# ArbiterMob/FluidSimulationCuda

Measured on AMD Instinct MI355X. Metric: Mcells/s per Jacobi iter, higher is better.
Workload: dtype f32

## Files before the change

### fluidsimulationcuda_amd/capi.py

```python
import ctypes as C
import os

import numpy as np

from ._build import LIB

OK, E_INVALID, E_NOMEM, E_HIP, E_COMM = 0, 1, 2, 3, 4
U, V, DENS, U_PREV, V_PREV, DENS_PREV, TMP0, TMP1, TMP2, TMP3, TMP4, TMP5 = range(12)
NFIELDS = 12
JACOBI_STREAM, JACOBI_LDS, JACOBI_NAIVE, JACOBI_TB = 0, 1, 2, 3
STORAGE_F32, STORAGE_F16 = 0, 1
PARAM_TB_MAX_SWEEPS, PARAM_TB_ROWS, PARAM_HALO, PARAM_TB_FAST_DIVISION, PARAM_TB_MIN_CELLS, PARAM_TB_EDGE_ROWS_PCT = 0, 1, 2, 3, 4, 5
PARAM_TB_LANE_COLUMNS = 6
PARAM_TB_T16_MIN_CELLS = 7
PARAM_TB_AUTOTUNE = 8
PARAM_FUSE_DIVERGENCE = 9
PARAM_SLAB_OVERLAP = 10
PARAM_EARLY_ADVECT = 11
PARAM_FUSE_ADD_SOURCE = 12
PARAM_XCHG_OVERLAP = 13
PARAM_F16_PRESSURE_SCALE = 14
XCHG_HALO, XCHG_GATHER, XCHG_MAX, XCHG_MAX_BEGIN, XCHG_MAX_END = 0, 1, 2, 3, 4
RCCL_ID_BYTES = 128
FIELD_NAMES = ("u", "v", "dens", "u_prev", "v_prev", "dens_prev", "tmp0", "tmp1", "tmp2", "tmp3", "tmp4", "tmp5")


class FluidError(RuntimeError):
    def __init__(self, code, msg):
        super().__init__("libfluid_amd error %d: %s" % (code, msg))
        self.code = code


class Config(C.Structure):
    _fields_ = [("n", C.c_int), ("rank", C.c_int), ("nranks", C.c_int), ("halo", C.c_int),
                ("jacobi_variant", C.c_int), ("stream", C.c_void_p), ("arena", C.c_void_p),
                ("arena_bytes", C.c_size_t), ("storage", C.c_int)]


TIME_SOURCE, TIME_DIFFUSION, TIME_DIVERGENCE, TIME_PROJECTION, TIME_ADVECTION = range(5)
TIMING_CATEGORIES = ("source", "diffusion", "divergence", "projection", "advection")


class Timing(C.Structure):
    _fields_ = [("jacobi_ms", C.c_double), ("sweeps", C.c_longlong), ("solves", C.c_longlong),
                ("category_ms", C.c_double * 5), ("category_calls", C.c_longlong * 5),
                ("jacobi_launches", C.c_longlong), ("jacobi_field_launches", C.c_longlong),
                ("pressure_ms", C.c_double), ("pressure_sweeps", C.c_longlong)]


EXCHANGE_FN = C.CFUNCTYPE(C.c_int, C.c_void_p, C.c_int, C.POINTER(C.c_int), C.c_int, C.c_int,
                          C.POINTER(C.c_float))

_HOSTF = np.ctypeslib.ndpointer(dtype=np.float32, flags="C_CONTIGUOUS")
_ctx = C.c_void_p
# ... 82 lines not shown
```

### fluidsimulationcuda_amd/csrc/fluid_ctx.h

```cpp
#pragma once
#include <hip/hip_runtime.h>

#include <string>
#include <vector>

#include "../../include/fluid_amd.h"
#include "fluid_kernels.h"

namespace fluid_detail {
int fail(int code, const char* fmt, ...);
int materialize_zero(fluid_ctx* c, int f);
struct RcclExchange;
void rccl_release(RcclExchange* x);
}

#define HIP_TRY(expr)                                                                                      \
    do {                                                                                                   \
        hipError_t e_ = (expr);                                                                            \
        if (e_ != hipSuccess)                                                                              \
            return fluid_detail::fail(e_ == hipErrorOutOfMemory ? FLUID_E_NOMEM : FLUID_E_HIP, "%s: %s",   \
                                      #expr, hipGetErrorString(e_));                                       \
    } while (0)

#define TRY(expr)                        \
// ... 14 lines not shown
};

struct fluid_ctx {
    int n = 0, w = 0, pitch = 0;
    size_t field_floats = 0;
    char* arena = nullptr;
    bool own_arena = false;
    int st = fluid::STORAGE_F32;
    size_t esz = 4;
    hipStream_t stream = nullptr;
    bool own_stream = false;
    hipStream_t stream2 = nullptr;
    hipEvent_t ev_fork = nullptr, ev_join = nullptr;
    bool slab_overlap = true;
    hipStream_t xstream = nullptr;
    hipEvent_t ev_xbegin = nullptr, ev_xdone = nullptr;
    bool xchg_overlap = true;
    unsigned xowed = 0;
    long long split_launches = 0;
    bool early_advect = true;
    float vmax_prev[2] = {-1.0f, -1.0f};
    FieldState field[FLUID_NFIELDS];
    size_t field_bytes = 0;
    unsigned int* d_scalar = nullptr;
    float* d_partials = nullptr;
    unsigned int* tiles = nullptr;
    unsigned int* h_scalar = nullptr;
    hipEvent_t scalar_ready = nullptr;
    int variant = fluid::JACOBI_TB;
    int tb_max_t = 16, tb_rows = 0, num_cu = 256;
    long long tb_min_cells = 0;
    long long tb_t16_min_cells = -1;
    bool fuse_divergence = true;
    bool autotune = true;
    struct Trial { unsigned long long key; int cand; hipEvent_t a, b; };
    std::vector<Trial> trials;
    std::vector<hipEvent_t> free_events;
    bool defer_zero_source = true;
    bool in_halo_exchange = false;
    int tb_nv = 2;
    int tb_edge_pct = 40;
    int fast_div = 2;
    int rank = 0, nranks = 1, own0 = 1, own1 = 1, min_slab = 0, halo = 1;
    bool fuse_add_source = true;
    float pscale = 1.0f;
    fluid_exchange_fn xchg = nullptr;
    void* xchg_user = nullptr;
    fluid_detail::RcclExchange* rccl = nullptr;
    bool timing = false;
    struct Ev { hipEvent_t a, b; int cat; bool pressure; };
    std::vector<Ev> ev_pool;
    size_t ev_used = 0;
    double cat_ms[FLUID_TIMING_CATEGORIES] = {};
    long long cat_calls[FLUID_TIMING_CATEGORIES] = {};
    long long sweeps = 0, pending_sweeps = 0, launches = 0, field_launches = 0;
    double pressure_ms = 0.0;
    long long pressure_sweeps = 0, pending_pressure_sweeps = 0;
    bool in_pressure_solve = false;

    bool valid_field(int id) const { return id >= 0 && id < FLUID_NFIELDS; }
    void* ptr(int id) const { return field[id].ptr; }
    void* row(int id, int r) const { return static_cast<char*>(ptr(id)) + (size_t)r * pitch * esz; }
    int lo_all() const { return own0 - (rank == 0 ? 1 : 0); }
    int hi_all() const { return own1 + (rank == nranks - 1 ? 1 : 0); }
};

// ... 1 lines not shown
```

### fluidsimulationcuda_amd/csrc/fluid_kernels.h

```cpp
#pragma once
#include <hip/hip_runtime.h>

namespace fluid {

constexpr int XOFF = 63;

enum JacobiVariant { JACOBI_STREAM = 0, JACOBI_LDS = 1, JACOBI_NAIVE = 2, JACOBI_TB = 3, JACOBI_VARIANTS = 4 };

enum Storage { STORAGE_F32 = 0, STORAGE_F16 = 1 };
typedef _Float16 half_t;
inline size_t storage_bytes(int st) { return st == STORAGE_F16 ? 2 : 4; }

inline int pitch_for(int n) { return ((XOFF + 1 + 4 * ((n + 3) / 4) + 1) + 63) / 64 * 64; }

struct TbBatch {
    const void* x[3];
    const void* x0[3];
    void* out[3];
    float alpha[3], beta[3];
    double yd[3];
    float hi[3], lo[3];
    const unsigned* tiles[3];
    unsigned tile_thr[3];
    int tile_pitch;
    void* div[3];
    float div_scale;
    int b[3];
    int x_zero[3];
    float x0_inc[3];
    int count;
};

void launch_set_bnd(hipStream_t s, int st, void* f, int pitch, int n, int b);
void launch_add_source(hipStream_t s, int st, void* x, const void* src, int pitch, int row_lo, int row_hi, float dt);
void launch_jacobi(hipStream_t s, int st, int variant, const void* x, const void* x0, void* out, int pitch, int n,
                   int row_lo, int row_hi, float alpha, float beta, int b);
void launch_jacobi_tb(hipStream_t s, int st, int T, int divmode, int nv, const TbBatch& batch, int pitch, int n, int row_lo,
                      int row_hi, int rb, int rb_edge, bool divsrc = false, bool addsrc = false, int hole_lo = 0, int hole_hi = 0);
inline bool jacobi_tb_addsrc_exists(int T, int divmode, int nv) { return nv == 2 && (T == 8 || T == 12 || T == 16) && (divmode == 0 || divmode == 2 || divmode == 5); }
constexpr int kTileRows = 32, kTileCols = 64;
inline int tile_rows(int n) { return (n + kTileRows - 1) / kTileRows; }
inline int tile_pitch(int n) { return (n + kTileCols - 1) / kTileCols; }
struct TileBatch {
    const void* field[3];
    unsigned* tiles[3];
};
void launch_tile_min_abs(hipStream_t s, int st, const TileBatch& tb, int count, int pitch, int n, int row_lo, int row_hi, int tile_pitch);
void launch_validate_div(hipStream_t s, int divmode, float beta, float kbeta, double yd, float hi, float lo, unsigned long long* bad);
void launch_advect(hipStream_t s, int st, void* d, const void* d0, const void* u, const void* v, int pitch, int n,
                   int row_lo, int row_hi, float dt0, int b);
void launch_advect2(hipStream_t s, int st, void* da, const void* d0a, int ba, void* db, const void* d0b, int bb, const void* u,
                    const void* v, int pitch, int n, int row_lo, int row_hi, float dt0);
void launch_divergence(hipStream_t s, int st, const void* u, const void* v, void* p, void* div, int pitch, int n,
                       int row_lo, int row_hi, float h, int write_p, float pscale = 1.0f);
void launch_scale(hipStream_t s, int st, void* x, int pitch, int row_lo, int row_hi, float factor);
constexpr int kMaxPartials = 8192;
void launch_subtract_gradient(hipStream_t s, int st, void* u, void* v, const void* p, int pitch, int n, int row_lo,
                              int row_hi, float h, float* partials = nullptr, unsigned int* max_out = nullptr, float pinv = 1.0f);
void launch_gradient_advect(hipStream_t s, int st, void* u, void* v, const void* p, void* d, const void* d0, int pitch, int n,
                            int row_lo, int row_hi, float h, float dt0, int b, float pinv = 1.0f);
void launch_absmax2(hipStream_t s, int st, const void* u, const void* v, int pitch, int n, int row_lo, int row_hi,
                    unsigned int* result);
void launch_residual(hipStream_t s, int st, const void* x, const void* x0, int pitch, int n, int row_lo, int row_hi,
                     float alpha, float beta, unsigned int* result);

}
```

### fluidsimulationcuda_amd/csrc/fluid_kernels.hip

```cpp
#include <hip/hip_runtime.h>
#include <stdint.h>

#include <algorithm>
#include <cstdlib>

#include "fluid_kernels.h"

namespace fluid {

__device__ __forceinline__ float flip_if(bool c, float v) { return c ? -v : v; }

__device__ __forceinline__ float keep_f32(float v) { asm("" : "+v"(v)); return v; }
__device__ __forceinline__ float ld1(const float* p) { return *p; }
__device__ __forceinline__ float ld1(const half_t* p) { return keep_f32((float)*p); }
__device__ __forceinline__ void st1(float* p, float v) { *p = v; }
__device__ __forceinline__ void st1(half_t* p, float v) { *p = (half_t)keep_f32(v); }
template <typename S>
__device__ __forceinline__ float as_stored(float v)
{
    if constexpr (sizeof(S) == 2) return keep_f32((float)(S)keep_f32(v));
    else return v;
}
typedef half_t half4_t __attribute__((ext_vector_type(4)));
__device__ __forceinline__ float4 ld4(const float* p) { return *reinterpret_cast<const float4*>(p); }
// ... 342 lines not shown
        __builtin_memcpy(&u, &h, 4);
        __builtin_amdgcn_raw_buffer_store_b32(u, r, off, 0, 0);
    }
}

struct DivK {
    float beta;
    double yd;
    float hi, lo;
};
constexpr float kDiv5NegScale = -0x1p24f;

template <typename S, int NV>
struct TbArgs {
    const S* xc;
    const S* rc;
    S* oc;
    __amdgpu_buffer_rsrc_t bx, br, bo;
    unsigned ld_off;
    unsigned st_off;
    unsigned row_bytes;
    unsigned m_lg;
    unsigned m_r[NV];
    int n, q_lo, q_hi, cg;
    float alpha;
    DivK k;
    S* dc;
    __amdgpu_buffer_rsrc_t bd;
    float div_scale;
    int s_lo, s_hi;
    unsigned sx, sy;
    float x0_inc;
    bool st_rg_lane, is_lg;
};

__device__ __forceinline__ float fxor(float v, unsigned m) { return __uint_as_float(__float_as_uint(v) ^ m); }
template <int NV>
__device__ __forceinline__ Vec<NV> fxorv(const Vec<NV>& v, unsigned m)
{
    Vec<NV> o;
#pragma unroll
    for (int c = 0; c < NV; ++c) o.c[c] = fxor(v.c[c], m);
    return o;
}

template <int DIVMODE>
__device__ __forceinline__ float tb_div(float num, const DivK& k)
{
    if (DIVMODE == 0) return num / k.beta;
    if (DIVMODE == 4) return num * k.beta;
    if (DIVMODE == 3) return __builtin_fmaf(num, k.hi, num * k.lo);
    if (DIVMODE == 5) {
        const float q0 = num * k.beta;
        const float e = __builtin_fmaf(q0, k.hi, num * kDiv5NegScale);
        return __builtin_fmaf(e, k.lo, q0);
    }
    return (float)((double)num * k.yd);
}
template <int DIVMODE>
__device__ __forceinline__ v2f tb_div2(v2f num, const DivK& k)
{
    if constexpr (DIVMODE == 4) return num * k.beta;
    else if constexpr (DIVMODE == 3) {
        const v2f p = num * k.lo;
        return __builtin_elementwise_fma(num, (v2f){k.hi, k.hi}, p);
    } else if constexpr (DIVMODE == 5) {
// ... 130 lines not shown

template <int NV>
__device__ __forceinline__ Vec<NV> take(const Vec<NV>& v)
{
    Vec<NV> o;
#pragma unroll
    for (int p = 0; p < NV; p += 2) {
        v2f in = {v.c[p], v.c[p + 1]}, out;
        asm("v_mov_b64 %0, %1" : "=v"(out) : "v"(in));
        o.c[p] = out.x;
        o.c[p + 1] = out.y;
    }
    return o;
}

template <int K, int N, int NV>
__device__ __forceinline__ void tb_qshift(Vec<NV> (&Q)[N])
{
    if constexpr (K >= 1) {
        Q[K] = Q[K - 1];
        tb_qshift<K - 1, N, NV>(Q);
    }
}

template <int DIVMODE, int NV>
__device__ __forceinline__ void tb_sticky(const Vec<NV>& G, v2f& nf)
{
    if constexpr (DIVMODE == 5) {
#pragma unroll
        for (int p = 0; p < NV; p += 2) nf = __builtin_elementwise_fma((v2f){G.c[p], G.c[p + 1]}, (v2f){0.f, 0.f}, nf);
    }
}

template <int T, int DIVMODE, bool EDGE, bool WALL, bool GEN, int PH, typename S, int NV, bool DIVSRC = false, bool ADDSRC = false>
__device__ __forceinline__ void tb_step(int t, Vec<NV> (&W)[T][3], Vec<NV> (&Q)[T + 1], Vec<NV> (&PX)[3], Vec<NV> (&PQ)[3],
                                        const TbArgs<S, NV>& a, Vec<NV> (&UR)[3], Vec<NV> (&VR)[3], v2f& nf)
{
    constexpr int UP = PH % 3, ME = (PH + 1) % 3, FR = (PH + 2) % 3;
    __builtin_amdgcn_sched_barrier(0);
    if constexpr (DIVSRC) {
        UR[FR] = take<NV>(PX[PH]);
        VR[FR] = take<NV>(PQ[PH]);
    } else {
        W[0][FR] = take<NV>(PX[PH]);
        Q[0] = take<NV>(PQ[PH]);
        if constexpr (ADDSRC) {
#pragma unroll
            for (int p = 0; p < NV; p += 2) {
                const v2f ds = (v2f){W[0][FR].c[p], W[0][FR].c[p + 1]} * a.div_scale;
                const v2f q = (v2f){Q[0].c[p], Q[0].c[p + 1]} + ds;
                Q[0].c[p] = as_stored<S>(q.x);
                Q[0].c[p + 1] = as_stored<S>(q.y);
            }
            buf_stv<NV>(a.dc, a.bd, (((t >= a.s_lo) & (t < a.s_hi)) ? a.st_off : kBufOff) + (unsigned)t * a.row_bytes, Q[0]);
        } else {
#pragma unroll
            for (int p = 0; p < NV; p += 2) {
                const v2f q = (v2f){Q[0].c[p], Q[0].c[p + 1]} + a.x0_inc;
                Q[0].c[p] = q.x;
                Q[0].c[p + 1] = q.y;
            }
        }
    }
    {
        const unsigned off = a.ld_off + (unsigned)(t + 3) * a.row_bytes;
        PX[PH] = buf_ldv<NV>(a.xc, a.bx, off);
        PQ[PH] = buf_ldv<NV>(a.rc, a.br, off);
    }
    __builtin_amdgcn_sched_barrier(0);
    if constexpr (DIVSRC) {
        const int q = t - 1;
        Vec<NV> D = tb_divergence<NV>(UR[ME], VR[UP], VR[FR], a.div_scale);
#pragma unroll
        for (int c = 0; c < NV; ++c) D.c[c] = as_stored<S>(D.c[c]);
        Q[1] = D;
        float v1 = 0.f, vn = 0.f;
        if (EDGE) tb_fix_columns<S, NV>(D, a, v1, vn, WALL);
        tb_store_to<EDGE, (WALL || GEN), S, NV>(a.dc, a.bd, D, q, (q >= 1) & (q <= a.n) & (q >= a.q_lo) & (q < a.q_hi), a, v1, vn);
    }
    if constexpr (!GEN) {
#pragma unroll
        for (int s = 1; s <= T; ++s) {
            const int q = t - s;
            Vec<NV> G = tb_stencil<DIVMODE, NV>(W[s - 1][UP], W[s - 1][ME], W[s - 1][FR], Q[s], a.alpha, a.k);
            float v1 = 0.f, vn = 0.f;
            if (EDGE) tb_fix_columns<S, NV>(G, a, v1, vn, WALL && s == T);
            if (s < T) W[s][FR] = G;
            else {
                tb_sticky<DIVMODE, NV>(G, nf);
                tb_store<EDGE, WALL, S, NV>(G, q, (q >= a.q_lo) & (q < a.q_hi), a, v1, vn);
            }
        }
    } else {
#pragma unroll
        for (int s = 1; s <= T; ++s) {
            const int q = t - s;
            const bool interior = (q >= 1 && q <= a.n);
            Vec<NV> G = tb_stencil<DIVMODE, NV>(W[s - 1][UP], W[s - 1][ME], W[s - 1][FR], Q[s], a.alpha, a.k);
            float v1 = 0.f, vn = 0.f;
            if (EDGE) tb_fix_columns<S, NV>(G, a, v1, vn, s == T);
            if (s < T) {
                const Vec<NV> me = W[s][ME];
                const Vec<NV> flipped_me = fxorv<NV>(me, a.sy);
                const Vec<NV> flipped_g = fxorv<NV>(G, a.sy);
                const bool bot_ghost = (q == a.n + 1), top_ghost = (q == 1);
#pragma unroll
                for (int c = 0; c < NV; ++c) {
                    W[s][FR].c[c] = bot_ghost ? flipped_me.c[c] : G.c[c];
                    W[s][ME].c[c] = top_ghost ? flipped_g.c[c] : me.c[c];
                }
            } else {
                tb_sticky<DIVMODE, NV>(G, nf);
                tb_store<EDGE, true, S, NV>(G, q, interior & (q >= a.q_lo) & (q < a.q_hi), a, v1, vn);
            }
        }
    }
    tb_qshift<T, T + 1, NV>(Q);
}

template <int T, int DIVMODE, bool EDGE, bool WALL, typename S, int NV, bool DIVSRC = false, bool ADDSRC = false>
__device__ __forceinline__ bool tb_march(int t0, int t1, const TbArgs<S, NV>& a)
{
    Vec<NV> W[T][3], Q[T + 1], PX[3], PQ[3], UR[3], VR[3];
    v2f nf = {0.f, 0.f};
    Vec<NV> zero;
#pragma unroll
    for (int c = 0; c < NV; ++c) zero.c[c] = 0.f;
#pragma unroll
    for (int s = 0; s < T; ++s) { W[s][0] = zero; W[s][1] = zero; W[s][2] = zero; }
#pragma unroll
    for (int s = 0; s <= T; ++s) Q[s] = zero;
#pragma unroll
    for (int d = 0; d < 3; ++d) { UR[d] = zero; VR[d] = zero; }
#pragma unroll
    for (int d = 0; d < 3; ++d) {
        const unsigned off = a.ld_off + (unsigned)(t0 + d) * a.row_bytes;
        PX[d] = buf_ldv<NV>(a.xc, a.bx, off);
        PQ[d] = buf_ldv<NV>(a.rc, a.br, off);
        buf_stv<NV>(a.oc, a.bo, kBufOff, zero);
        if constexpr (DIVSRC || ADDSRC) buf_stv<NV>(a.dc, a.bd, kBufOff, zero);
        __builtin_amdgcn_sched_barrier(0);
    }
    int t = t0;
    if constexpr (WALL) {
        for (; t <= t1 && t < T + 1; t += 3) {
            tb_step<T, DIVMODE, EDGE, WALL, true, 0, S, NV, DIVSRC, ADDSRC>(t, W, Q, PX, PQ, a, UR, VR, nf);
            tb_step<T, DIVMODE, EDGE, WALL, true, 1, S, NV, DIVSRC, ADDSRC>(t + 1, W, Q, PX, PQ, a, UR, VR, nf);
            tb_step<T, DIVMODE, EDGE, WALL, true, 2, S, NV, DIVSRC, ADDSRC>(t + 2, W, Q, PX, PQ, a, UR, VR, nf);
        }
    }
    for (; t <= t1 && (!WALL || t + 1 <= a.n); t += 3) {
        tb_step<T, DIVMODE, EDGE, WALL, false, 0, S, NV, DIVSRC, ADDSRC>(t, W, Q, PX, PQ, a, UR, VR, nf);
        tb_step<T, DIVMODE, EDGE, WALL, false, 1, S, NV, DIVSRC, ADDSRC>(t + 1, W, Q, PX, PQ, a, UR, VR, nf);
        tb_step<T, DIVMODE, EDGE, WALL, false, 2, S, NV, DIVSRC, ADDSRC>(t + 2, W, Q, PX, PQ, a, UR, VR, nf);
    }
    if constexpr (WALL) {
        for (; t <= t1; t += 3) {
            tb_step<T, DIVMODE, EDGE, WALL, true, 0, S, NV, DIVSRC, ADDSRC>(t, W, Q, PX, PQ, a, UR, VR, nf);
            tb_step<T, DIVMODE, EDGE, WALL, true, 1, S, NV, DIVSRC, ADDSRC>(t + 1, W, Q, PX, PQ, a, UR, VR, nf);
            tb_step<T, DIVMODE, EDGE, WALL, true, 2, S, NV, DIVSRC, ADDSRC>(t + 2, W, Q, PX, PQ, a, UR, VR, nf);
        }
    }
    if constexpr (DIVMODE == 5) return __builtin_amdgcn_ballot_w64((nf.x != nf.x) | (nf.y != nf.y)) != 0ull;
    else return false;
}

template <int T, int DIVMODE, typename S, int NV, bool DIVSRC = false, bool ADDSRC = false>
__device__ __forceinline__ bool tb_march_any(bool edge, bool wall, int t0, int t1, const TbArgs<S, NV>& a)
{
    if (edge) {
        if (wall) return tb_march<T, DIVMODE, true, true, S, NV, DIVSRC, ADDSRC>(t0, t1, a);
        return tb_march<T, DIVMODE, true, false, S, NV, DIVSRC, ADDSRC>(t0, t1, a);
    }
    if (wall) return tb_march<T, DIVMODE, false, true, S, NV, DIVSRC, ADDSRC>(t0, t1, a);
    return tb_march<T, DIVMODE, false, false, S, NV, DIVSRC, ADDSRC>(t0, t1, a);
}

struct TbGrid {
    int inner_wins, inner_blocks, edge_wins, edge_blocks, first_right;
    int hole_lo, hole_hi;
};

constexpr int tb_waves_per_simd(int T, int NV) { return NV == 2 ? (T <= 8 ? 4 : T <= 12 ? 3 : 2) : (T <= 4 ? 3 : 2); }

template <int T, int DIVMODE, int NV, typename S, bool DIVSRC = false, bool ADDSRC = false>
__global__ __launch_bounds__(256, tb_waves_per_simd(T, NV)) void k_jacobi_tb(TbBatch batch, int pitch, int n, int row_lo,
                                                                             int row_hi, int rb, int rb_edge, TbGrid g)
{
    static_assert(!DIVSRC || DIVMODE == 4, "the divergence-sourced launch is the first launch of a pressure solve");
    static_assert(!(DIVSRC && ADDSRC) && (!ADDSRC || DIVMODE != 3), "one second store per launch; mode 3's tiles are taken from the summed field");
    const unsigned per_xcd = gridDim.x >> 3;
    unsigned vid = (blockIdx.x & 7u) * per_xcd + (blockIdx.x >> 3);
    if (vid >= (unsigned)(g.inner_blocks + g.edge_blocks)) return;
    int win, strip_group;
    if (vid < (unsigned)g.inner_blocks) {
        win = 1 + (int)(vid % (unsigned)g.inner_wins);
        strip_group = (int)(vid / (unsigned)g.inner_wins);
    } else {
        vid -= (unsigned)g.inner_blocks;
        const int e = (int)(vid % (unsigned)g.edge_wins);
        strip_group = (int)(vid / (unsigned)g.edge_wins);
        win = e == 0 ? 0 : g.first_right + e - 1;
    }
    const S* __restrict__ x = static_cast<const S*>(batch.x[blockIdx.z]);
    const S* __restrict__ x0 = static_cast<const S*>(batch.x0[blockIdx.z]);
    S* __restrict__ out = static_cast<S*>(batch.out[blockIdx.z]);
    const float alpha = batch.alpha[blockIdx.z], beta = batch.beta[blockIdx.z];
    const double yd = batch.yd[blockIdx.z];
    const int b = batch.b[blockIdx.z];
    constexpr int HL = (T + NV - 1) / NV;
    constexpr int VS = 64 - 2 * HL;
    constexpr int C0 = (XOFF + 1) / NV;
    static_assert((XOFF + 1) % NV == 0 && HL <= C0, "window overlap must fit the row's left pad");
    const int lane = threadIdx.x & 63;
    const int strip = strip_group * 4 + __builtin_amdgcn_readfirstlane(threadIdx.x >> 6);
    const int kg = n / NV;
    const bool left_edge = (win == 0);
    const bool right_edge = (kg >= win * VS - HL) && (kg < win * VS - HL + 64);
    const bool edge = left_edge || right_edge;
    const int rbw = edge ? rb_edge : rb;
// ... 18 lines not shown
    const bool ld_ok = k <= pitch / NV - C0 - 1;
    const ptrdiff_t cofs = (ptrdiff_t)(XOFF + 1) + NV * (ptrdiff_t)(ld_ok ? k : 0);
    a.xc = x + cofs;
    a.rc = x0 + cofs;
    a.oc = out + cofs;
    {
        const unsigned field_bytes = (unsigned)((size_t)(n + 2) * (size_t)pitch * sizeof(S));
        a.bx = __builtin_amdgcn_make_buffer_rsrc(const_cast<S*>(x), 0, (batch.x_zero[blockIdx.z] && !DIVSRC) ? 0u : field_bytes, 0x00020000);
        a.br = __builtin_amdgcn_make_buffer_rsrc(const_cast<S*>(x0), 0, field_bytes, 0x00020000);
        a.bo = __builtin_amdgcn_make_buffer_rsrc(out, 0, field_bytes, 0x00020000);
        S* dv = (DIVSRC || ADDSRC) ? static_cast<S*>(batch.div[blockIdx.z]) : out;
        a.dc = dv + cofs;
        a.bd = __builtin_amdgcn_make_buffer_rsrc(dv, 0, field_bytes, 0x00020000);
        a.div_scale = batch.div_scale;
        a.row_bytes = (unsigned)((size_t)pitch * sizeof(S));
        const unsigned col = (unsigned)((XOFF + 1 + NV * (ptrdiff_t)k) * (ptrdiff_t)sizeof(S));
        a.ld_off = ld_ok ? col : kBufOff;
    }
    a.n = n;
    a.cg = n % NV;
    a.is_lg = (k == -1);
    const bool is_rg = (k == kg);
    const bool own = (lane >= HL) && (lane < 64 - HL);
    const bool st_int = own && k >= 0 && k < nvec;
    a.st_rg_lane = is_rg && (own || k == nvec);
    a.m_lg = a.is_lg ? 0xFFFFFFFFu : 0u;
#pragma unroll
    for (int c = 0; c < NV; ++c) a.m_r[c] = (is_rg && a.cg == c) ? 0xFFFFFFFFu : 0u;
    a.st_off = (ld_ok && (st_int || a.is_lg || a.st_rg_lane)) ? a.ld_off : kBufOff;
    a.sx = (b == 1) ? 0x80000000u : 0u;
    a.sy = (b == 2) ? 0x80000000u : 0u;
    a.alpha = alpha;
    a.k.beta = beta;
    const int t0 = max(0, a.q_lo - T), t1 = a.q_hi - 1 + T;
    const bool wall = (a.q_lo < T) || (a.q_hi - 1 + T > n + 1);
    constexpr int DM = DIVMODE == 3 ? 2 : DIVMODE;
    bool two_term = false;
    if constexpr (DIVMODE == 3) {
        const unsigned* __restrict__ tiles = batch.tiles[blockIdx.z];
        const unsigned thr = batch.tile_thr[blockIdx.z];
        const int tr0 = (max(1, a.q_lo - T + 1) - 1) / kTileRows, tr1 = (min(n, a.q_hi + T - 2) - 1) / kTileRows;
        const int c0 = max(1, 1 + NV * (win * VS - HL)), c1 = min(n, NV * (win * VS - HL + 64));
        const int tc0 = (c0 - 1) / kTileCols, tc1 = (c1 - 1) / kTileCols, ntc = tc1 - tc0 + 1;
        const int count = (tr1 - tr0 + 1) * ntc;
        bool low = false;
        if (tiles != nullptr)
            for (int i = lane; i < count; i += 64)
                low |= tiles[(size_t)(tr0 + i / ntc) * batch.tile_pitch + (tc0 + i % ntc)] < thr;
        two_term = tiles != nullptr && __builtin_amdgcn_ballot_w64(low) == 0ull;
    }
    if (two_term) {
        tb_march_any<T, DIVMODE, S, NV>(edge, wall, t0, t1, a);
    } else {
        const bool again = tb_march_any<T, DM, S, NV, DIVSRC, ADDSRC>(edge, wall, t0, t1, a);
        if constexpr (DIVMODE == 5) {
            if (again) tb_march_any<T, 2, S, NV, false, ADDSRC>(edge, wall, t0, t1, a);
        }
    }
}

template <typename S>
__global__ __launch_bounds__(256) void k_tile_min_abs(TileBatch tb, int pitch, int n, int row_lo, int row_hi, int tile_row0, int tile_pitch)
{
    const S* __restrict__ f = static_cast<const S*>(tb.field[blockIdx.z]);
    unsigned* __restrict__ out = tb.tiles[blockIdx.z];
    const int lane = threadIdx.x & 63, wave = threadIdx.x >> 6;
// ... 392 lines not shown
{
    const size_t total = (size_t)(row_hi - row_lo) * (pitch >> 2);
    const unsigned blocks = (unsigned)((total + 255) / 256 < 8192 ? (total + 255) / 256 : 8192);
    FLUID_BY_STORAGE(st, hipLaunchKernelGGL(k_scale<S>, dim3(blocks ? blocks : 1), dim3(256), 0, s, (S*)x, pitch, row_lo, row_hi, factor));
}

void launch_jacobi(hipStream_t s, int st, int variant, const void* x, const void* x0, void* out, int pitch, int n,
                   int row_lo, int row_hi, float alpha, float beta, int b)
{
    const int rows = row_hi - row_lo;
    if (rows <= 0) return;
    switch (variant) {
    case JACOBI_NAIVE:
        FLUID_BY_STORAGE(st, hipLaunchKernelGGL(k_jacobi_naive<S>, dim3(cdiv(n, 64), cdiv(rows, 4)), dim3(256), 0, s,
                                                (const S*)x, (const S*)x0, (S*)out, pitch, n, row_lo, row_hi, alpha,
                                                beta, b));
        break;
    case JACOBI_LDS:
        FLUID_BY_STORAGE(st, hipLaunchKernelGGL(k_jacobi_lds<S>, dim3(cdiv(n, LT_X), cdiv(rows, LT_Y)), dim3(256), 0, s,
                                                (const S*)x, (const S*)x0, (S*)out, pitch, n, row_lo, row_hi, alpha,
                                                beta, b));
        break;
    default: {
        constexpr int RB = 8;
        const unsigned nvec = (n + 3) / 4;
        FLUID_BY_STORAGE(st, hipLaunchKernelGGL((k_jacobi_stream<RB, S>), dim3(cdiv(nvec, 256), cdiv(rows, RB)), dim3(256),
                                                0, s, (const S*)x, (const S*)x0, (S*)out, pitch, n, row_lo, row_hi,
                                                alpha, beta, b));
    }
    }
}

void launch_jacobi_tb(hipStream_t s, int st, int T, int divmode, int nv, const TbBatch& batch, int pitch, int n, int row_lo,
                      int row_hi, int rb, int rb_edge, bool divsrc, bool addsrc, int hole_lo, int hole_hi)
{
    const int rows = row_hi - row_lo;
    if (rows <= 0 || batch.count <= 0) return;
    if (hole_lo < row_lo) hole_lo = row_lo;
    if (hole_hi > row_hi) hole_hi = row_hi;
    const bool hole = hole_lo < hole_hi;
    if (hole && hole_lo == row_lo && hole_hi == row_hi) return;
    if (T == 16 || T == 12) nv = 2;
    const int HL = (T + nv - 1) / nv, VS = 64 - 2 * HL;
    const unsigned nvec = (n + nv - 1) / nv;
    rb_edge = rb_edge < 1 ? rb : (rb_edge > rb ? rb : rb_edge);
    const int nwin = (int)cdiv(nvec, VS), kg = n / nv;
    int first_right = nwin - 1;
    while (first_right > 1 && kg < (first_right - 1) * VS - HL + 64) --first_right;
    if (first_right < 1) first_right = 1;
    TbGrid g;
    g.first_right = first_right;
    g.inner_wins = first_right - 1;
    g.edge_wins = 1 + (nwin - first_right);
    auto strips = [&](int r) { return hole ? cdiv(hole_lo - row_lo, r) + cdiv(row_hi - hole_hi, r) : cdiv(rows, r); };
    g.hole_lo = hole ? hole_lo : 0;
    g.hole_hi = hole ? hole_hi : 0;
    g.inner_blocks = g.inner_wins * (int)cdiv(strips(rb), 4);
    g.edge_blocks = g.edge_wins * (int)cdiv(strips(rb_edge), 4);
    const dim3 grid(8 * cdiv(g.inner_blocks + g.edge_blocks, 8), 1, batch.count), block(256);
#define FLUID_TB2(TT, DD, NN) \
    FLUID_BY_STORAGE(st, hipLaunchKernelGGL((k_jacobi_tb<TT, DD, NN, S>), grid, block, 0, s, batch, pitch, n, row_lo, row_hi, rb, rb_edge, g))
#define FLUID_TB1(TT, DD)            \
    if (nv == 2) FLUID_TB2(TT, DD, 2); \
    else FLUID_TB2(TT, DD, 4)
#define FLUID_TB(TT)                          \
    if (divmode == 4) { FLUID_TB1(TT, 4); }      \
    else if (divmode == 5) { FLUID_TB1(TT, 5); } \
    else if (divmode == 3) { FLUID_TB1(TT, 3); } \
    else if (divmode == 2) { FLUID_TB1(TT, 2); } \
    else { FLUID_TB1(TT, 0); }
#define FLUID_TBD(TT) \
    FLUID_BY_STORAGE(st, hipLaunchKernelGGL((k_jacobi_tb<TT, 4, 2, S, true>), grid, block, 0, s, batch, pitch, n, row_lo, row_hi, rb, rb_edge, g))
#define FLUID_TBA2(TT, DD) \
    FLUID_BY_STORAGE(st, hipLaunchKernelGGL((k_jacobi_tb<TT, DD, 2, S, false, true>), grid, block, 0, s, batch, pitch, n, row_lo, row_hi, rb, rb_edge, g))
#define FLUID_TBA(TT)                       \
    if (divmode == 5) { FLUID_TBA2(TT, 5); }      \
    else if (divmode == 2) { FLUID_TBA2(TT, 2); } \
    else { FLUID_TBA2(TT, 0); }
    if (addsrc) {
        if (T == 16) { FLUID_TBA(16) }
        else if (T == 12) { FLUID_TBA(12) }
        else { FLUID_TBA(8) }
    }
    else if (divsrc) {
        if (T == 16) { FLUID_TBD(16); }
        else if (T == 12) { FLUID_TBD(12); }
        else { FLUID_TBD(8); }
    }
    else if (T == 16) {
        if (divmode == 4) { FLUID_TB2(16, 4, 2); }
        else if (divmode == 5) { FLUID_TB2(16, 5, 2); }
        else if (divmode == 3) { FLUID_TB2(16, 3, 2); }
        else if (divmode == 2) { FLUID_TB2(16, 2, 2); }
        else { FLUID_TB2(16, 0, 2); }
    }
    else if (T == 12) {
        if (divmode == 4) { FLUID_TB2(12, 4, 2); }
        else if (divmode == 5) { FLUID_TB2(12, 5, 2); }
        else if (divmode == 3) { FLUID_TB2(12, 3, 2); }
        else if (divmode == 2) { FLUID_TB2(12, 2, 2); }
        else { FLUID_TB2(12, 0, 2); }
    }
    else if (T == 8) { FLUID_TB(8) }
    else if (T == 4) { FLUID_TB(4) }
    else { FLUID_TB(2) }
#undef FLUID_TBA
#undef FLUID_TBA2
// ... 113 lines not shown
```

### fluidsimulationcuda_amd/csrc/fluid_solver.hip

```cpp
#include <hip/hip_runtime.h>

#include <algorithm>
#include <cmath>
#include <cstdarg>
#include <cstdio>
#include <cstring>
#include <functional>
#include <mutex>
#include <new>
#include <string>
#include <unordered_map>
#include <vector>

#include "fluid_ctx.h"

namespace fluid_detail {

thread_local std::string g_err;

int fail(int code, const char* fmt, ...)
{
    char buf[512];
    va_list ap;
    va_start(ap, fmt);
// ... 352 lines not shown
            c->field[x].src_dt = dt;
            return FLUID_OK;
        }
        TIMED(c, FLUID_TIME_SOURCE, fluid::launch_add_source(c->stream, c->st, c->ptr(x), c->ptr(s), c->pitch, lo, hi, dt));
    }
    wrote(c, x, reach);
    return FLUID_OK;
}

struct RbTuner {
    struct Entry {
        std::vector<int> cand;
        std::vector<float> best_ms;
        std::vector<int> samples, issued;
        int fixed = 0;
    };
    std::mutex mu;
    std::unordered_map<unsigned long long, Entry> table;
};
RbTuner& rb_tuner()
{
    static RbTuner t;
    return t;
}
constexpr int kTuneSamples = 2;

unsigned long long tune_key(const fluid_ctx* c, int T, int m, int divmode, long long rows_n)
{
    int dev = 0;
    (void)hipGetDevice(&dev);
    unsigned long long h = 1469598103934665603ull;
    for (unsigned long long v : {(unsigned long long)dev, (unsigned long long)c->n, (unsigned long long)rows_n, (unsigned long long)T,
                                 (unsigned long long)m, (unsigned long long)divmode, (unsigned long long)c->tb_nv, (unsigned long long)c->st,
                                 (unsigned long long)c->tb_edge_pct}) {
        h ^= v;
        h *= 1099511628211ull;
    }
    return h;
}

void tune_harvest(fluid_ctx* c)
{
    if (c->trials.empty()) return;
    RbTuner& t = rb_tuner();
    std::lock_guard<std::mutex> lock(t.mu);
    size_t keep = 0;
    for (size_t k = 0; k < c->trials.size(); ++k) {
        fluid_ctx::Trial& tr = c->trials[k];
        if (hipEventQuery(tr.b) != hipSuccess) {
            c->trials[keep++] = tr;
            continue;
        }
        float ms = 0.f;
        auto it = t.table.find(tr.key);
        if (hipEventElapsedTime(&ms, tr.a, tr.b) == hipSuccess && it != t.table.end() && !it->second.fixed) {
            RbTuner::Entry& e = it->second;
            e.best_ms[tr.cand] = e.samples[tr.cand] ? std::min(e.best_ms[tr.cand], ms) : ms;
            e.samples[tr.cand] += 1;
            bool done = true;
            for (int sdone : e.samples) done = done && sdone >= kTuneSamples;
            if (done) {
                e.fixed = e.cand[std::min_element(e.best_ms.begin(), e.best_ms.end()) - e.best_ms.begin()];
                if (std::getenv("FLUID_TUNE_LOG")) {
                    std::string msg;
                    for (size_t q = 0; q < e.cand.size(); ++q) msg += " " + std::to_string(e.cand[q]) + ":" + std::to_string((int)(e.best_ms[q] * 1e3f));
                    fprintf(stderr, "[fluid tune] key %016llx -> %d rows  (height:us%s)\n", tr.key, e.fixed, msg.c_str());
                }
            }
        }
        c->free_events.push_back(tr.a);
        c->free_events.push_back(tr.b);
    }
    c->trials.resize(keep);
}

int tune_pick(fluid_ctx* c, unsigned long long key, int heuristic, int T, long long rows_n, int* trial)
{
    *trial = -1;
    tune_harvest(c);
    RbTuner& t = rb_tuner();
    std::lock_guard<std::mutex> lock(t.mu);
    RbTuner::Entry& e = t.table[key];
    if (e.fixed) return e.fixed;
    if (e.cand.empty()) {
        e.cand.push_back(heuristic);
        for (int r : {48, 56, 64, 80, 96, 112, 128, 160, 192}) {
            if (r < 2 * T || r >= rows_n + 2 * T) continue;
            if (std::find(e.cand.begin(), e.cand.end(), r) == e.cand.end()) e.cand.push_back(r);
        }
        if (rows_n <= 2200)
            for (int r : {2, 4, 8, 12, 24, 32, 40})
                if (r < rows_n && std::find(e.cand.begin(), e.cand.end(), r) == e.cand.end()) e.cand.push_back(r);
        if (e.cand.size() == 1) {
            e.fixed = heuristic;
            return heuristic;
        }
        e.best_ms.assign(e.cand.size(), 0.f);
        e.samples.assign(e.cand.size(), 0);
        e.issued.assign(e.cand.size(), 0);
    }
    const int pick = (int)(std::min_element(e.issued.begin(), e.issued.end()) - e.issued.begin());
    if (e.issued[pick] >= kTuneSamples + 2) return e.cand[0];
    e.issued[pick] += 1;
    *trial = pick;
    return e.cand[pick];
}

int tune_begin(fluid_ctx* c, unsigned long long key, int trial)
{
    fluid_ctx::Trial tr{};
    tr.key = key;
    tr.cand = trial;
    for (hipEvent_t* ev : {&tr.a, &tr.b}) {
        if (!c->free_events.empty()) {
            *ev = c->free_events.back();
            c->free_events.pop_back();
        } else {
            HIP_TRY(hipEventCreate(ev));
        }
    }
    HIP_TRY(hipEventRecord(tr.a, c->stream));
    c->trials.push_back(tr);
// ... 184 lines not shown
        bt.yd[q] = p.yd;
        bt.hi[q] = p.hi;
        bt.lo[q] = p.lo;
        bt.tiles[q] = p.mode == 3 ? solve_tiles(c, B.scratch_base + j) : nullptr;
        bt.tile_thr[q] = p.tile_thr;
        bt.b[q] = B.sv[j].b;
        bt.x_zero[q] = c->field[B.cur[j]].zero ? 1 : 0;
        bt.x0_inc[q] = x0.pend && !addsrc && !divsrc ? x0.pend_inc : -0.0f;
        if (addsrc) bt.div[q] = c->ptr(B.sum[j]);
    }
    bt.count = last - first;
    bt.tile_pitch = fluid::tile_pitch(c->n);
    if (addsrc) bt.div_scale = c->field[B.sv[first].x0].src_dt;
    if (divsrc) {
        bt.x[0] = c->ptr(B.ds->u);
        bt.x0[0] = c->ptr(B.ds->v);
        bt.div[0] = c->ptr(B.sv[0].x0);
        bt.div_scale = B.ds->scale;
    }
    return bt;
}

int edge_rows(const fluid_ctx* c, int T, int rb) { return std::max(2 * T, rb * (c->tb_edge_pct > 0 ? c->tb_edge_pct : 100) / 100); }

int strip_rows(const fluid_ctx* c, int T, int m, long long rows_n)
{
    const int nv = c->tb_nv;
    const int HL = (T + nv - 1) / nv, VS = 64 - 2 * HL;
    const long long windows = ((c->n + nv - 1) / nv + VS - 1) / VS;
    const long long inner = windows > 2 ? windows - 2 : 0, outer = windows - inner;
    const int resident = nv == 2 ? (T >= 16 ? 2 : 4) : (T >= 8 ? 2 : 3);
    const long long room = (long long)c->num_cu * resident * 92 / 100;
    const int cap = T >= 16 ? 192 : (T >= 8 ? 80 : 96) * (m > 1 ? 2 : 1);
    int rb = 2 * T;
    for (; rb < cap; rb += 2) {
        const long long si = (rows_n + rb - 1) / rb, se = (rows_n + edge_rows(c, T, rb) - 1) / edge_rows(c, T, rb);
        if ((inner * ((si + 3) / 4) + outer * ((se + 3) / 4)) * m <= room) break;
    }
    if (rows_n <= 1100) rb = std::max(2, std::min(rb, (int)(rows_n / 64) & ~1));
    return rb;
}

int launch_fused(fluid_ctx* c, const fluid::TbBatch& bt, int T, int divmode, bool divsrc, bool addsrc, int lo, int hi)
{
    const bool owed = c->nranks > 1 && (c->xowed & stream_bit(c));
    const int in_lo = owed && c->rank > 0 ? std::max(lo, c->own0 + T) : lo;
    const int in_hi = owed && c->rank < c->nranks - 1 ? std::min(hi, c->own1 - T) : hi;
    const bool split = owed && in_hi - in_lo >= 2 * T && (in_lo > lo || in_hi < hi);
    for (int part = split ? 0 : 1; part < 2; ++part) {
        const int plo = part ? lo : in_lo, phi = part ? hi : in_hi;
        const int hole_lo = part && split ? in_lo : 0, hole_hi = part && split ? in_hi : 0;
        if (part) TRY(xchg_join(c));
        const long long rows_n = (phi - plo) - std::max(0, hole_hi - hole_lo);
        int rb = c->tb_rows > 0 ? c->tb_rows : strip_rows(c, T, bt.count, rows_n);
        int trial = -1;
        unsigned long long key = 0;
        if (c->tb_rows <= 0 && c->autotune) {
            key = tune_key(c, T, bt.count + (divsrc ? 8 : 0) + (addsrc ? 16 : 0) + (hole_hi > hole_lo ? 32 : 0), divmode, rows_n);
            rb = tune_pick(c, key, rb, T, rows_n, &trial);
        }
        if (trial >= 0) TRY(tune_begin(c, key, trial));
        fluid::launch_jacobi_tb(c->stream, c->st, T, divmode, c->tb_nv, bt, c->pitch, c->n, plo, phi, rb, std::min(rb, edge_rows(c, T, rb)),
                                divsrc, addsrc, hole_lo, hole_hi);
        if (trial >= 0) TRY(tune_end(c));
    }
    if (split) c->split_launches += 1;
    return FLUID_OK;
}

void commit_launch(fluid_ctx* c, Batch& B, bool first, int r)
{
    if (B.ds && first && c->nranks > 1)
        c->field[B.sv[0].x0].reach = std::max(0, std::min(c->field[B.sv[0].x0].reach, r));
    if (B.add_src && first) {
        for (int j = 0; j < B.count; ++j) {
            trade(c, B.sv[j].x0, B.sum[j]);
            wrote(c, B.sum[j], 0);
            wrote(c, B.sv[j].x0, std::max(0, r));
        }
        B.add_src = false;
    }
    for (int j = 0; j < B.count; ++j) {
        c->field[B.cur[j]].zero = false;
        wrote(c, B.nxt[j], r);
        std::swap(B.cur[j], B.nxt[j]);
    }
}

int batch_sweep(fluid_ctx* c, Batch& B)
{
    const Solve* sv = B.sv;
    const bool multi = c->nranks > 1, canonical = B.shape.canonical;
    int r = multi ? batch_reach(c, B) : kEverywhere;
    for (int k = 0; k < B.iters;) {
        const int remaining = B.iters - k;
        const int wantT = canonical ? pick_sweeps(c, remaining, remaining, B.shape, B.all_mode4) : 1;
// ... 679 lines not shown
    TRY(check_ctx(c));
    if (variant < 0 || variant >= fluid::JACOBI_VARIANTS) return fail(FLUID_E_INVALID, "unknown Jacobi variant %d", variant);
    c->variant = variant;
    return FLUID_OK;
}

int fluid_set_param(fluid_ctx* c, int key, int value)
{
    TRY(check_ctx(c));
    switch (key) {
    case FLUID_PARAM_TB_MAX_SWEEPS:
        if (value != 16 && value != 12 && value != 8 && value != 4 && value != 2) return fail(FLUID_E_INVALID, "TB_MAX_SWEEPS must be 16, 12, 8, 4 or 2");
        c->tb_max_t = value;
        return FLUID_OK;
    case FLUID_PARAM_TB_ROWS:
        if (value < 0) return fail(FLUID_E_INVALID, "TB_ROWS must be >= 0");
        c->tb_rows = value;
        return FLUID_OK;
    case FLUID_PARAM_TB_EDGE_ROWS_PCT:
        if (value < 0 || value > 100) return fail(FLUID_E_INVALID, "TB_EDGE_ROWS_PCT must be in [0,100]");
        c->tb_edge_pct = value;
        return FLUID_OK;
    case FLUID_PARAM_TB_MIN_CELLS:
        if (value < 0) return fail(FLUID_E_INVALID, "TB_MIN_CELLS must be >= 0");
        c->tb_min_cells = value;
        return FLUID_OK;
    case FLUID_PARAM_TB_FAST_DIVISION:
        if (value < 0 || value > 3) return fail(FLUID_E_INVALID, "TB_FAST_DIVISION must be 0, 1, 2 or 3");
        c->fast_div = value;
        return FLUID_OK;
    case FLUID_PARAM_TB_AUTOTUNE:
        c->autotune = value != 0;
        return FLUID_OK;
    case FLUID_PARAM_SLAB_OVERLAP:
        c->slab_overlap = value != 0;
        return FLUID_OK;
    case FLUID_PARAM_FUSE_DIVERGENCE:
        c->fuse_divergence = value != 0;
        return FLUID_OK;
    case FLUID_PARAM_EARLY_ADVECT:
        c->early_advect = value != 0;
        return FLUID_OK;
    case FLUID_PARAM_FUSE_ADD_SOURCE:
        c->fuse_add_source = value != 0;
        return FLUID_OK;
    case FLUID_PARAM_F16_PRESSURE_SCALE: {
        for (int f = 0; f < FLUID_NFIELDS; ++f) TRY(unscale(c, f));
        int e = 0;
        (void)std::frexp((float)c->n, &e);
        c->pscale = (value != 0 && c->st == fluid::STORAGE_F16 && c->n >= 16) ? std::ldexp(1.0f, e - 3) : 1.0f;
        return FLUID_OK;
    }
    case FLUID_PARAM_XCHG_OVERLAP:
        TRY(xchg_join(c));
        c->xchg_overlap = value != 0;
        return FLUID_OK;
    case FLUID_PARAM_TB_T16_MIN_CELLS:
        if (value < -1) return fail(FLUID_E_INVALID, "TB_T16_MIN_CELLS must be >= 0, or -1 for the default rule");
        c->tb_t16_min_cells = value;
        return FLUID_OK;
    case FLUID_PARAM_TB_LANE_COLUMNS:
        if (value != 2 && value != 4) return fail(FLUID_E_INVALID, "TB_LANE_COLUMNS must be 2 or 4");
        c->tb_nv = value;
        return FLUID_OK;
    case FLUID_PARAM_HALO:
        if (value < 1) return fail(FLUID_E_INVALID, "HALO must be >= 1");
// ... 334 lines not shown
```

### include/fluid_amd.h

```cpp
#ifndef FLUID_AMD_H
#define FLUID_AMD_H

#include <stddef.h>

#ifdef __cplusplus
extern "C" {
#endif

#define FLUID_OK        0
#define FLUID_E_INVALID 1
#define FLUID_E_NOMEM   2
#define FLUID_E_HIP     3
#define FLUID_E_COMM    4

enum {
    FLUID_U = 0, FLUID_V = 1, FLUID_DENS = 2,
    FLUID_U_PREV = 3, FLUID_V_PREV = 4, FLUID_DENS_PREV = 5,
    FLUID_TMP0 = 6, FLUID_TMP1 = 7, FLUID_TMP2 = 8,
    FLUID_TMP3 = 9, FLUID_TMP4 = 10, FLUID_TMP5 = 11,
    FLUID_NFIELDS = 12
};

enum { FLUID_JACOBI_STREAM = 0, FLUID_JACOBI_LDS = 1, FLUID_JACOBI_NAIVE = 2, FLUID_JACOBI_TB = 3 };

enum {
    FLUID_PARAM_TB_MAX_SWEEPS = 0,
    FLUID_PARAM_TB_ROWS = 1,
    FLUID_PARAM_HALO = 2,
    FLUID_PARAM_TB_FAST_DIVISION = 3
    ,FLUID_PARAM_TB_EDGE_ROWS_PCT = 5
    ,FLUID_PARAM_TB_LANE_COLUMNS = 6
    ,FLUID_PARAM_TB_T16_MIN_CELLS = 7
    ,FLUID_PARAM_TB_AUTOTUNE = 8
    ,FLUID_PARAM_SLAB_OVERLAP = 10
    ,FLUID_PARAM_EARLY_ADVECT = 11
    ,FLUID_PARAM_FUSE_DIVERGENCE = 9
    ,FLUID_PARAM_FUSE_ADD_SOURCE = 12
    ,FLUID_PARAM_XCHG_OVERLAP = 13
    ,FLUID_PARAM_F16_PRESSURE_SCALE = 14
    ,FLUID_PARAM_TB_MIN_CELLS = 4
};

typedef struct fluid_ctx fluid_ctx;

const char *fluid_last_error(void);

int step(int N, float dt, float diff, float visc, float *u, float *v, float *dens);
int step_src(int N, float dt, float diff, float visc, int iters,
             float *u, float *v, float *dens,
             float *u_prev, float *v_prev, float *dens_prev);
int fluid_release_cached(void);

int fluid_coefficients(int N, float dt, float coef, float *alpha, float *beta);

typedef struct fluid_config {
    int n;
    int rank, nranks;
    int halo;
    int jacobi_variant;
    void *stream;
    void *arena;
    size_t arena_bytes;
    int storage;
} fluid_config;

enum { FLUID_STORAGE_F32 = 0, FLUID_STORAGE_F16 = 1 };

size_t fluid_arena_bytes(int N);
size_t fluid_arena_bytes_ex(int N, int storage);
int fluid_layout(int N, int *pitch, int *xoff, size_t *field_floats);

int fluid_create(int N, fluid_ctx **out);
// ... 83 lines not shown
```

Before: 4.037 million.

## Skip idle pipeline stages during temporal-blocking fill and drain phases

Adds a partial-stage path to the temporally blocked Jacobi kernel. During the pipeline fill at the start of a strip and the drain at its end, stencil stages that have no valid input yet are skipped instead of computed and discarded. Because shorter strips now waste less work, the minimum rows per block drops from 2T to T and the autotuner gains smaller candidates, giving more blocks and better occupancy on large grids. The change adds extra unrolled loop copies, which raises code size and register pressure, and the fill/drain stage arithmetic has to be exact for results to stay correct.

```diff
diff --git a/fluidsimulationcuda_amd/capi.py b/fluidsimulationcuda_amd/capi.py
--- a/fluidsimulationcuda_amd/capi.py
+++ b/fluidsimulationcuda_amd/capi.py
@@ -20,6 +20,7 @@
 PARAM_FUSE_ADD_SOURCE = 12
 PARAM_XCHG_OVERLAP = 13
 PARAM_F16_PRESSURE_SCALE = 14
+PARAM_TB_FILL = 15
 XCHG_HALO, XCHG_GATHER, XCHG_MAX, XCHG_MAX_BEGIN, XCHG_MAX_END = 0, 1, 2, 3, 4
 RCCL_ID_BYTES = 128
 FIELD_NAMES = ("u", "v", "dens", "u_prev", "v_prev", "dens_prev", "tmp0", "tmp1", "tmp2", "tmp3", "tmp4", "tmp5")
diff --git a/fluidsimulationcuda_amd/csrc/fluid_ctx.h b/fluidsimulationcuda_amd/csrc/fluid_ctx.h
--- a/fluidsimulationcuda_amd/csrc/fluid_ctx.h
+++ b/fluidsimulationcuda_amd/csrc/fluid_ctx.h
@@ -70,6 +70,7 @@
     long long tb_min_cells = 0;
     long long tb_t16_min_cells = -1;
     bool fuse_divergence = true;
+    bool tb_fill = true;
     bool autotune = true;
     struct Trial { unsigned long long key; int cand; hipEvent_t a, b; };
     std::vector<Trial> trials;
diff --git a/fluidsimulationcuda_amd/csrc/fluid_kernels.h b/fluidsimulationcuda_amd/csrc/fluid_kernels.h
--- a/fluidsimulationcuda_amd/csrc/fluid_kernels.h
+++ b/fluidsimulationcuda_amd/csrc/fluid_kernels.h
@@ -36,7 +36,8 @@
 void launch_jacobi(hipStream_t s, int st, int variant, const void* x, const void* x0, void* out, int pitch, int n,
                    int row_lo, int row_hi, float alpha, float beta, int b);
 void launch_jacobi_tb(hipStream_t s, int st, int T, int divmode, int nv, const TbBatch& batch, int pitch, int n, int row_lo,
-                      int row_hi, int rb, int rb_edge, bool divsrc = false, bool addsrc = false, int hole_lo = 0, int hole_hi = 0);
+                      int row_hi, int rb, int rb_edge, bool divsrc = false, bool addsrc = false, int hole_lo = 0, int hole_hi = 0,
+                      bool fill = true);
 inline bool jacobi_tb_addsrc_exists(int T, int divmode, int nv) { return nv == 2 && (T == 8 || T == 12 || T == 16) && (divmode == 0 || divmode == 2 || divmode == 5); }
 constexpr int kTileRows = 32, kTileCols = 64;
 inline int tile_rows(int n) { return (n + kTileRows - 1) / kTileRows; }
diff --git a/fluidsimulationcuda_amd/csrc/fluid_kernels.hip b/fluidsimulationcuda_amd/csrc/fluid_kernels.hip
--- a/fluidsimulationcuda_amd/csrc/fluid_kernels.hip
+++ b/fluidsimulationcuda_amd/csrc/fluid_kernels.hip
@@ -398,6 +398,7 @@
     unsigned sx, sy;
     float x0_inc;
     bool st_rg_lane, is_lg;
+    bool fill;
 };
 
 __device__ __forceinline__ float fxor(float v, unsigned m) { return __uint_as_float(__float_as_uint(v) ^ m); }
@@ -594,10 +595,12 @@
     }
 }
 
-template <int T, int DIVMODE, bool EDGE, bool WALL, bool GEN, int PH, typename S, int NV, bool DIVSRC = false, bool ADDSRC = false>
+template <int T, int DIVMODE, bool EDGE, bool WALL, bool GEN, int PH, typename S, int NV, bool DIVSRC = false, bool ADDSRC = false,
+          bool PART = false>
 __device__ __forceinline__ void tb_step(int t, Vec<NV> (&W)[T][3], Vec<NV> (&Q)[T + 1], Vec<NV> (&PX)[3], Vec<NV> (&PQ)[3],
-                                        const TbArgs<S, NV>& a, Vec<NV> (&UR)[3], Vec<NV> (&VR)[3], v2f& nf)
-{
+                                        const TbArgs<S, NV>& a, Vec<NV> (&UR)[3], Vec<NV> (&VR)[3], v2f& nf, int smax = T)
+{
+    static_assert(!(PART && GEN), "the general body runs every stage");
     constexpr int UP = PH % 3, ME = (PH + 1) % 3, FR = (PH + 2) % 3;
     __builtin_amdgcn_sched_barrier(0);
     if constexpr (DIVSRC) {
@@ -643,15 +646,20 @@
     if constexpr (!GEN) {
 #pragma unroll
         for (int s = 1; s <= T; ++s) {
+            const bool run = !PART || s <= smax;
             const int q = t - s;
-            Vec<NV> G = tb_stencil<DIVMODE, NV>(W[s - 1][UP], W[s - 1][ME], W[s - 1][FR], Q[s], a.alpha, a.k);
+            Vec<NV> G;
             float v1 = 0.f, vn = 0.f;
-            if (EDGE) tb_fix_columns<S, NV>(G, a, v1, vn, WALL && s == T);
+            if (run) {
+                G = tb_stencil<DIVMODE, NV>(W[s - 1][UP], W[s - 1][ME], W[s - 1][FR], Q[s], a.alpha, a.k);
+                if (EDGE) tb_fix_columns<S, NV>(G, a, v1, vn, WALL && s == T);
+                if (s == T) tb_sticky<DIVMODE, NV>(G, nf);
+            } else {
+#pragma unroll
+                for (int c = 0; c < NV; ++c) G.c[c] = __builtin_nondeterministic_value(W[s - 1][FR].c[c]);
+            }
             if (s < T) W[s][FR] = G;
-            else {
-                tb_sticky<DIVMODE, NV>(G, nf);
-                tb_store<EDGE, WALL, S, NV>(G, q, (q >= a.q_lo) & (q < a.q_hi), a, v1, vn);
-            }
+            else tb_store<EDGE, WALL, S, NV>(G, q, run & (q >= a.q_lo) & (q < a.q_hi), a, v1, vn);
         }
     } else {
 #pragma unroll
@@ -711,10 +719,23 @@
             tb_step<T, DIVMODE, EDGE, WALL, true, 2, S, NV, DIVSRC, ADDSRC>(t + 2, W, Q, PX, PQ, a, UR, VR, nf);
         }
     }
-    for (; t <= t1 && (!WALL || t + 1 <= a.n); t += 3) {
+    const int fill_end = (a.fill && t0 == a.q_lo - T) ? t0 + 3 * ((2 * T + 2) / 3) : t0;
+    const int full_end = a.fill ? t1 - 2 : t1;
+    auto stages = [&](int u) { return u > t1 ? 0 : u < fill_end ? (u - t0) >> 1 : T; };
+    for (; t <= t1 && t < fill_end && (!WALL || t + 1 <= a.n); t += 3) {
+        tb_step<T, DIVMODE, EDGE, WALL, false, 0, S, NV, DIVSRC, ADDSRC, true>(t, W, Q, PX, PQ, a, UR, VR, nf, stages(t));
+        tb_step<T, DIVMODE, EDGE, WALL, false, 1, S, NV, DIVSRC, ADDSRC, true>(t + 1, W, Q, PX, PQ, a, UR, VR, nf, stages(t + 1));
+        tb_step<T, DIVMODE, EDGE, WALL, false, 2, S, NV, DIVSRC, ADDSRC, true>(t + 2, W, Q, PX, PQ, a, UR, VR, nf, stages(t + 2));
+    }
+    for (; t <= full_end && (!WALL || t + 1 <= a.n); t += 3) {
         tb_step<T, DIVMODE, EDGE, WALL, false, 0, S, NV, DIVSRC, ADDSRC>(t, W, Q, PX, PQ, a, UR, VR, nf);
         tb_step<T, DIVMODE, EDGE, WALL, false, 1, S, NV, DIVSRC, ADDSRC>(t + 1, W, Q, PX, PQ, a, UR, VR, nf);
         tb_step<T, DIVMODE, EDGE, WALL, false, 2, S, NV, DIVSRC, ADDSRC>(t + 2, W, Q, PX, PQ, a, UR, VR, nf);
+    }
+    for (; t <= t1 && (!WALL || t + 1 <= a.n); t += 3) {
+        tb_step<T, DIVMODE, EDGE, WALL, false, 0, S, NV, DIVSRC, ADDSRC, true>(t, W, Q, PX, PQ, a, UR, VR, nf, stages(t));
+        tb_step<T, DIVMODE, EDGE, WALL, false, 1, S, NV, DIVSRC, ADDSRC, true>(t + 1, W, Q, PX, PQ, a, UR, VR, nf, stages(t + 1));
+        tb_step<T, DIVMODE, EDGE, WALL, false, 2, S, NV, DIVSRC, ADDSRC, true>(t + 2, W, Q, PX, PQ, a, UR, VR, nf, stages(t + 2));
     }
     if constexpr (WALL) {
         for (; t <= t1; t += 3) {
@@ -747,7 +768,7 @@
 
 template <int T, int DIVMODE, int NV, typename S, bool DIVSRC = false, bool ADDSRC = false>
 __global__ __launch_bounds__(256, tb_waves_per_simd(T, NV)) void k_jacobi_tb(TbBatch batch, int pitch, int n, int row_lo,
-                                                                             int row_hi, int rb, int rb_edge, TbGrid g)
+                                                                             int row_hi, int rb, int rb_edge, TbGrid g, int fill)
 {
     static_assert(!DIVSRC || DIVMODE == 4, "the divergence-sourced launch is the first launch of a pressure solve");
     static_assert(!(DIVSRC && ADDSRC) && (!ADDSRC || DIVMODE != 3), "one second store per launch; mode 3's tiles are taken from the summed field");
@@ -832,6 +853,7 @@
     a.sy = (b == 2) ? 0x80000000u : 0u;
     a.alpha = alpha;
     a.k.beta = beta;
+    a.fill = fill != 0;
     const int t0 = max(0, a.q_lo - T), t1 = a.q_hi - 1 + T;
     const bool wall = (a.q_lo < T) || (a.q_hi - 1 + T > n + 1);
     constexpr int DM = DIVMODE == 3 ? 2 : DIVMODE;
@@ -1290,7 +1312,7 @@
 }
 
 void launch_jacobi_tb(hipStream_t s, int st, int T, int divmode, int nv, const TbBatch& batch, int pitch, int n, int row_lo,
-                      int row_hi, int rb, int rb_edge, bool divsrc, bool addsrc, int hole_lo, int hole_hi)
+                      int row_hi, int rb, int rb_edge, bool divsrc, bool addsrc, int hole_lo, int hole_hi, bool fill)
 {
     const int rows = row_hi - row_lo;
     if (rows <= 0 || batch.count <= 0) return;
@@ -1317,7 +1339,7 @@
     g.edge_blocks = g.edge_wins * (int)cdiv(strips(rb_edge), 4);
     const dim3 grid(8 * cdiv(g.inner_blocks + g.edge_blocks, 8), 1, batch.count), block(256);
 #define FLUID_TB2(TT, DD, NN) \
-    FLUID_BY_STORAGE(st, hipLaunchKernelGGL((k_jacobi_tb<TT, DD, NN, S>), grid, block, 0, s, batch, pitch, n, row_lo, row_hi, rb, rb_edge, g))
+    FLUID_BY_STORAGE(st, hipLaunchKernelGGL((k_jacobi_tb<TT, DD, NN, S>), grid, block, 0, s, batch, pitch, n, row_lo, row_hi, rb, rb_edge, g, fill ? 1 : 0))
 #define FLUID_TB1(TT, DD)            \
     if (nv == 2) FLUID_TB2(TT, DD, 2); \
     else FLUID_TB2(TT, DD, 4)
@@ -1328,9 +1350,9 @@
     else if (divmode == 2) { FLUID_TB1(TT, 2); } \
     else { FLUID_TB1(TT, 0); }
 #define FLUID_TBD(TT) \
-    FLUID_BY_STORAGE(st, hipLaunchKernelGGL((k_jacobi_tb<TT, 4, 2, S, true>), grid, block, 0, s, batch, pitch, n, row_lo, row_hi, rb, rb_edge, g))
+    FLUID_BY_STORAGE(st, hipLaunchKernelGGL((k_jacobi_tb<TT, 4, 2, S, true>), grid, block, 0, s, batch, pitch, n, row_lo, row_hi, rb, rb_edge, g, fill ? 1 : 0))
 #define FLUID_TBA2(TT, DD) \
-    FLUID_BY_STORAGE(st, hipLaunchKernelGGL((k_jacobi_tb<TT, DD, 2, S, false, true>), grid, block, 0, s, batch, pitch, n, row_lo, row_hi, rb, rb_edge, g))
+    FLUID_BY_STORAGE(st, hipLaunchKernelGGL((k_jacobi_tb<TT, DD, 2, S, false, true>), grid, block, 0, s, batch, pitch, n, row_lo, row_hi, rb, rb_edge, g, fill ? 1 : 0))
 #define FLUID_TBA(TT)                       \
     if (divmode == 5) { FLUID_TBA2(TT, 5); }      \
     else if (divmode == 2) { FLUID_TBA2(TT, 2); } \
diff --git a/fluidsimulationcuda_amd/csrc/fluid_solver.hip b/fluidsimulationcuda_amd/csrc/fluid_solver.hip
--- a/fluidsimulationcuda_amd/csrc/fluid_solver.hip
+++ b/fluidsimulationcuda_amd/csrc/fluid_solver.hip
@@ -408,7 +408,7 @@
     unsigned long long h = 1469598103934665603ull;
     for (unsigned long long v : {(unsigned long long)dev, (unsigned long long)c->n, (unsigned long long)rows_n, (unsigned long long)T,
                                  (unsigned long long)m, (unsigned long long)divmode, (unsigned long long)c->tb_nv, (unsigned long long)c->st,
-                                 (unsigned long long)c->tb_edge_pct}) {
+                                 (unsigned long long)c->tb_edge_pct, (unsigned long long)c->tb_fill}) {
         h ^= v;
         h *= 1099511628211ull;
     }
@@ -461,9 +461,12 @@
     if (e.cand.empty()) {
         e.cand.push_back(heuristic);
         for (int r : {48, 56, 64, 80, 96, 112, 128, 160, 192}) {
-            if (r < 2 * T || r >= rows_n + 2 * T) continue;
+            if (r < T || r >= rows_n + 2 * T) continue;
             if (std::find(e.cand.begin(), e.cand.end(), r) == e.cand.end()) e.cand.push_back(r);
         }
+        if (rows_n > 2200)
+            for (int r : {32, 40})
+                if (r >= T && std::find(e.cand.begin(), e.cand.end(), r) == e.cand.end()) e.cand.push_back(r);
         if (rows_n <= 2200)
             for (int r : {2, 4, 8, 12, 24, 32, 40})
                 if (r < rows_n && std::find(e.cand.begin(), e.cand.end(), r) == e.cand.end()) e.cand.push_back(r);
@@ -714,7 +717,7 @@
     const int resident = nv == 2 ? (T >= 16 ? 2 : 4) : (T >= 8 ? 2 : 3);
     const long long room = (long long)c->num_cu * resident * 92 / 100;
     const int cap = T >= 16 ? 192 : (T >= 8 ? 80 : 96) * (m > 1 ? 2 : 1);
-    int rb = 2 * T;
+    int rb = c->tb_fill ? T : 2 * T;
     for (; rb < cap; rb += 2) {
         const long long si = (rows_n + rb - 1) / rb, se = (rows_n + edge_rows(c, T, rb) - 1) / edge_rows(c, T, rb);
         if ((inner * ((si + 3) / 4) + outer * ((se + 3) / 4)) * m <= room) break;
@@ -743,7 +746,7 @@
         }
         if (trial >= 0) TRY(tune_begin(c, key, trial));
         fluid::launch_jacobi_tb(c->stream, c->st, T, divmode, c->tb_nv, bt, c->pitch, c->n, plo, phi, rb, std::min(rb, edge_rows(c, T, rb)),
-                                divsrc, addsrc, hole_lo, hole_hi);
+                                divsrc, addsrc, hole_lo, hole_hi, c->tb_fill);
         if (trial >= 0) TRY(tune_end(c));
     }
     if (split) c->split_launches += 1;
@@ -1489,6 +1492,9 @@
     case FLUID_PARAM_TB_AUTOTUNE:
         c->autotune = value != 0;
         return FLUID_OK;
+    case FLUID_PARAM_TB_FILL:
+        c->tb_fill = value != 0;
+        return FLUID_OK;
     case FLUID_PARAM_SLAB_OVERLAP:
         c->slab_overlap = value != 0;
         return FLUID_OK;
diff --git a/include/fluid_amd.h b/include/fluid_amd.h
--- a/include/fluid_amd.h
+++ b/include/fluid_amd.h
@@ -38,6 +38,7 @@
     ,FLUID_PARAM_FUSE_ADD_SOURCE = 12
     ,FLUID_PARAM_XCHG_OVERLAP = 13
     ,FLUID_PARAM_F16_PRESSURE_SCALE = 14
+    ,FLUID_PARAM_TB_FILL = 15
     ,FLUID_PARAM_TB_MIN_CELLS = 4
 };
 
```

New measurement: 4.253 million, median of 6. 1.05x the previous value.
